# ska-sa/dc_sand

Measured on AMD Instinct MI355X. Metric: Gcoeff/s (complex weights) 64ant x 1024beam x 32768chan per GPU, higher is better.
Workload: dtype f32

## Files before the change

dc_sand_amd/csrc/bf_beamform_i8_kernel.inc:

```
#ifndef BF_I8_WEIGHTED
#define BF_I8_WEIGHTED 0
#endif
#ifndef BF_I8_QUANT
#define BF_I8_QUANT 0
#endif
#ifndef BF_I8_POWER
#define BF_I8_POWER 0
#endif
template <int FORM, bool FULL, int NW = 4>
__global__ void __launch_bounds__(NW * 64) __attribute__((amdgpu_waves_per_eu(i8_waves_per_eu(FORM, FULL, BF_I8_QUANT))))
#if BF_I8_WEIGHTED && BF_I8_POWER
bf_beamform_i8_wp_kernel(const bf_bacc_args a, const bf_weights_args w)
#elif BF_I8_POWER
bf_beamform_i8_p_kernel(const bf_bacc_args a)
#elif BF_I8_WEIGHTED && BF_I8_QUANT
bf_beamform_i8_wq_kernel(const bf_bacc_args a, const bf_weights_args w, const bf_quant_args qa)
#elif BF_I8_QUANT
bf_beamform_i8_q_kernel(const bf_bacc_args a, const bf_quant_args qa)
#elif BF_I8_WEIGHTED
bf_beamform_i8_w_kernel(const bf_bacc_args a, const bf_weights_args w)
#else
bf_beamform_i8_kernel(const bf_bacc_args a)
#endif
{
    constexpr bool WEIGHTED = BF_I8_WEIGHTED, QUANT = BF_I8_QUANT;
#if !BF_I8_WEIGHTED
    const bf_weights_args w{};
#endif
#if !BF_I8_QUANT
    const bf_quant_args qa{};
#endif
    static_assert(NW == 4 || ((NW == 8 || NW == 16) && FORM == kStaged), "8- and 16-wave workgroups exist for the staged form only");
    static_assert(!WEIGHTED || FORM == kStaged || FORM == kChain, "weights exist for the product's forms only");
    static_assert(!QUANT || (NW == 4 && (FORM == kStaged || FORM == kChain)), "the quantiser exists for the product's forms only");
    static_assert(!BF_I8_POWER || (!BF_I8_QUANT && NW == 4 && (FORM == kStaged || FORM == kChain)), "the detector exists for the product's forms only");
    constexpr bool STAGED = FORM == kStaged, SPLIT = FORM == kSplit, CHAIN = FORM == kChain;
    extern __shared__ __attribute__((aligned(16))) char staged[];
    uint32_t bid = BACC_LOGICAL_ID(a);
    const uint32_t wave = __builtin_amdgcn_readfirstlane(threadIdx.x >> 6);
    const uint32_t lane = threadIdx.x & 63u;
    const uint32_t bg = bid % a.n_bgroups;
    bid /= a.n_bgroups;
    const uint32_t tg = bid % a.n_tgroups;
    const uint32_t c = bid / a.n_tgroups;
    const uint32_t nbt_log2 = SPLIT || CHAIN ? 0u : a.nbt_log2;
    const uint32_t nbt = 1u << nbt_log2, tpr = SPLIT ? 1u : (uint32_t)NW >> nbt_log2;
    const uint32_t bt = SPLIT ? 0u : wave & (nbt - 1u), slot = SPLIT ? 0u : wave >> nbt_log2;
    const uint32_t kc = SPLIT || CHAIN ? wave : 0u;
    const uint32_t lm = lane & 15u, lg = lane >> 4;
    const uint32_t bw = (bg * nbt + bt) * 16u;
    const uint32_t tt0 = tg * a.tiles_per_wg;
    const uint32_t tt1 = min(tt0 + a.tiles_per_wg, a.nT16);
    const uint32_t n_blocks = tt1 > tt0 + slot ? (tt1 - tt0 - slot + tpr - 1u) / tpr : 0u;
    const bool idle = bw >= a.B || n_blocks == 0u;
    if (!STAGED && !CHAIN && idle) return;
    const bool has_chunk = !(SPLIT || CHAIN) || 64u * kc < a.A;
    if (STAGED) {
        typedef __attribute__((address_space(3))) void lds_void;
        typedef const __attribute__((address_space(1))) void glb_void;
        const uint32_t bytes = (tt1 - tt0) * a.A * 32u;
        const char *src = reinterpret_cast<const char *>(a.ant) + ((uint64_t)c * a.nT16 + tt0) * a.A * 32u;
        for (uint32_t k = wave; k * 1024u < bytes; k += (uint32_t)NW)
            __builtin_amdgcn_global_load_lds((glb_void *)(src + min(k * 1024u + lane * 16u, bytes - 16u)), (lds_void *)(staged + k * 1024u),
                                             16, 0, 0);
    }

    const uint32_t fw = a.flags[0];
    const uint32_t cls = (fw >> 2) == a.epoch ? (fw & 3u) : DCS_CLASS_FAST_LOW;
    const float fChan = (float)c;
    const float D = a.k.fDenominator, y = a.k.fRcpDenominator;
    const float inv = 1.0f / kFixScale;
    float fac[4] = {inv, inv, inv, inv};
    if constexpr (WEIGHTED && STAGED) {
#pragma unroll
        for (int r = 0; r < 4; r++) fac[r] = w.gs[min(bw + (lane >> 4) + 4u * (uint32_t)r, a.B - 1u)] * inv;
    } else if constexpr (WEIGHTED && CHAIN) {
        fac[0] = w.gs[min(bw + (lane & 15u), a.B - 1u)] * inv;
    }
    float kq[4] = {0.0f, 0.0f, 0.0f, 0.0f};
    uint32_t n_clip = 0u;
    if constexpr (QUANT && STAGED) {
#pragma unroll
        for (int r = 0; r < 4; r++) kq[r] = qa.gains[min(bw + (lane >> 4) + 4u * (uint32_t)r, a.B - 1u)];
    }

    const bool shared_w = STAGED && a.share_off != 0u && tpr > 1u && cls != DCS_CLASS_SLOW;
    intx4 wre[3], wim[3];
#pragma unroll
    for (int d = 0; d < 3; d++) wre[d] = wim[d] = intx4{0, 0, 0, 0};
    bool bad_re = false, bad_im = false;
    auto make_coefficients = [&]() {
        const uint32_t beam = bw + 4u * (lm & 3u) + (lm >> 2);
        const bool beam_live = beam < a.B;
        const float *tp = a.terms + 2u * (uint64_t)min(beam, a.B - 1u);
        const float *gp = WEIGHTED ? w.gn + min(beam, a.B - 1u) : nullptr;
        auto planes = [](const uint32_t (&g)[4], uint32_t (&out)[3]) {
            const uint32_t t0 = __builtin_amdgcn_perm(g[1], g[0], 0x05010400u), t1 = __builtin_amdgcn_perm(g[1], g[0], 0x07030602u);
            const uint32_t t2 = __builtin_amdgcn_perm(g[3], g[2], 0x05010400u), t3 = __builtin_amdgcn_perm(g[3], g[2], 0x07030602u);
            out[2] = __builtin_amdgcn_perm(t2, t0, 0x05040100u);
            out[1] = __builtin_amdgcn_perm(t2, t0, 0x07060302u);
            out[0] = __builtin_amdgcn_perm(t3, t1, 0x05040100u);
        };
        auto four = [&](auto gen, auto track, uint32_t q, const floatx2 (&k4)[4], const float (&g4)[4], uint32_t (&nr)[3],
                        uint32_t (&ni)[3]) {
            uint32_t gr[4], gi[4];
#pragma unroll
            for (uint32_t z = 0; z < 4; z++) {
                float re, im;
                gen(k4[z].x, k4[z].y, re, im);
                if constexpr (WEIGHTED) re = g4[z] * re, im = g4[z] * im;
                if (decltype(track)::value) {
                    bad_re |= !(fabsf(re) <= 2.0f);
                    bad_im |= !(fabsf(im) <= 2.0f);
                }
                gr[z] = fixed_word(re), gi[z] = fixed_word(im);
            }
            planes(gr, nr), planes(gi, ni);
            if (!FULL) {
                uint32_t mask = 0;
#pragma unroll
                for (uint32_t z = 0; z < 4; z++) mask |= 64u * kc + 4u * (4u * q + z) + lg < a.A ? 0xffu << (8u * z) : 0u;
#pragma unroll
                for (int d = 0; d < 3; d++) nr[d] &= mask, ni[d] &= mask;
            }
        };
// ... 2 lines not shown
            float gw[16];
#pragma unroll
            for (uint32_t z = 0; z < 16; z++) {
                const uint32_t ant = 64u * kc + 4u * z + lg;
                if constexpr (WEIGHTED) {
                    if (decltype(unrolled)::value && z >= 4u) continue;
                    gw[z] = gp[(uint64_t)min(ant, a.A - 1u) * a.B];
                }
                kp[z] = *reinterpret_cast<const floatx2 *>(tp + 2u * (uint64_t)min(ant, a.A - 1u) * a.B);
            }
            if (decltype(unrolled)::value) {
#pragma unroll
                for (uint32_t q = 0; q < 4; q++) {
                    if constexpr (WEIGHTED) {
                        if (q < 3u) {
#pragma unroll
                            for (uint32_t z = 4u * q + 4u; z < 4u * q + 8u; z++) {
                                const uint32_t ant = 64u * kc + 4u * z + lg;
                                gw[z] = gp[(uint64_t)min(ant, a.A - 1u) * a.B];
                                kp[z] = *reinterpret_cast<const floatx2 *>(tp + 2u * (uint64_t)min(ant, a.A - 1u) * a.B);
                            }
                        }
                    }
                    if (shared_w && (q & (tpr - 1u)) != slot) continue;
                    const floatx2 k4[4] = {kp[4 * q], kp[4 * q + 1], kp[4 * q + 2], kp[4 * q + 3]};
                    float g4[4] = {};
                    if constexpr (WEIGHTED) g4[0] = gw[4 * q], g4[1] = gw[4 * q + 1], g4[2] = gw[4 * q + 2], g4[3] = gw[4 * q + 3];
                    uint32_t nr[3], ni[3];
                    four(gen, std::false_type{}, q, k4, g4, nr, ni);
                    if constexpr (CHAIN) {
                        uint32_t *cw = reinterpret_cast<uint32_t *>(staged) + (kc * 6u * 64u + lane) * 4u + q;
#pragma unroll
                        for (int d = 0; d < 3; d++) cw[(uint32_t)d * 256u] = beam_live ? nr[d] : 0u, cw[(3u + (uint32_t)d) * 256u] = beam_live ? ni[d] : 0u;
                    } else {
#pragma unroll
                        for (int d = 0; d < 3; d++) wre[d][q] = (int)nr[d], wim[d][q] = (int)ni[d];
                    }
                }
            } else {
#pragma unroll 1
                for (uint32_t q = 0; q < 4; q++) {
                    const floatx2 k4[4] = {kp[0], kp[1], kp[2], kp[3]};
                    float g4[4] = {};
                    if constexpr (WEIGHTED) {
#pragma unroll
                        for (uint32_t z = 0; z < 4; z++) g4[z] = gp[(uint64_t)min(64u * kc + 4u * (4u * q + z) + lg, a.A - 1u) * a.B];
                    }
                    uint32_t nr[3], ni[3];
                    four(gen, std::true_type{}, q, k4, g4, nr, ni);
                    if constexpr (CHAIN) {
                        uint32_t *cw = reinterpret_cast<uint32_t *>(staged) + (kc * 6u * 64u + lane) * 4u + q;
#pragma unroll
                        for (int d = 0; d < 3; d++) cw[(uint32_t)d * 256u] = beam_live ? nr[d] : 0u, cw[(3u + (uint32_t)d) * 256u] = beam_live ? ni[d] : 0u;
                    } else {
#pragma unroll
                        for (int d = 0; d < 3; d++) {
                            wre[d] = intx4{wre[d][1], wre[d][2], wre[d][3], (int)nr[d]};
                            wim[d] = intx4{wim[d][1], wim[d][2], wim[d][3], (int)ni[d]};
                        }
                    }
#pragma unroll
                    for (uint32_t z = 0; z < 12; z++) kp[z] = kp[z + 4];
                }
            }
            if (!CHAIN && !beam_live) {
#pragma unroll
                for (int d = 0; d < 3; d++) wre[d] = wim[d] = intx4{0, 0, 0, 0};
            }
        };
        if (cls == DCS_CLASS_SLOW) {
            generate([&](float kx, float ky, float &re, float &im) { coeff_slow(kx, ky, fChan, D, re, im); }, std::false_type{});
        } else {
            dispatch_fast(a.k.uDiv3Exact != 0u, cls == DCS_CLASS_FAST_LOW, [&](auto div3, auto lowdeg) {
                generate([&](float kx, float ky, float &re, float &im) {
                    coeff_fast<decltype(div3)::value, decltype(lowdeg)::value>(kx, ky, fChan, D, y, re, im);
                }, std::true_type{});
            });
        }
    };

    const char *ant8 = reinterpret_cast<const char *>(a.ant);
    const uint32_t blk_bytes = a.A * 32u;
    const uint32_t m = lm & 7u;
    const bool second = lm >= 8u;
    const uint32_t last = n_blocks - 1u;
    const uint32_t voff = lg * 32u + m * 4u;
    uint32_t cur[2][16];
    auto arrived = [&](uint32_t (&v)[16]) {
        asm volatile("" : "+v"(v[0]), "+v"(v[1]), "+v"(v[2]), "+v"(v[3]), "+v"(v[4]), "+v"(v[5]), "+v"(v[6]), "+v"(v[7]));
        asm volatile("" : "+v"(v[8]), "+v"(v[9]), "+v"(v[10]), "+v"(v[11]), "+v"(v[12]), "+v"(v[13]), "+v"(v[14]), "+v"(v[15]));
    };
    auto fetch = [&](uint32_t (&dst)[16], uint32_t blk, uint32_t kc) {
        const uint32_t blkA = min(blk, last), blkB = min(blk + 1u, last);
        if (STAGED) {
            const uint32_t at = ((second ? blkB : blkA) * tpr + slot) * blk_bytes + m * 4u;
#pragma unroll
            for (uint32_t p = 0; p < 16; p++)
                dst[p] = *reinterpret_cast<const uint32_t *>(staged + at + (FULL ? lg + 4u * p : min(lg + 4u * p, a.A - 1u)) * 32u);
// ... 179 lines not shown
        } else {
            for (uint32_t blk = 0; blk < n_blocks; blk += 4) {
                if (has_chunk) {
                    arrived(cur[0]);
                    arrived(cur[1]);
#pragma unroll
                    for (int h = 0; h < 2; h++) {
                        intx4 x[4];
                        floatx4 f[4];
                        transpose(cur[h], x);
                        contract(x, f);
                        if (SPLIT)
                            park(h, f);
                        else
                            finish(whole, blk + 2u * h, f);
                    }
                }
                if (SPLIT) {
                    __syncthreads();
                    gather(whole, 0, blk);
                    gather(whole, 1, blk + 2u);
                    __syncthreads();
                }
                __builtin_amdgcn_sched_barrier(0);
                if (has_chunk) {
                    fetch(cur[0], blk + 4u, kc);
                    fetch(cur[1], blk + 6u, kc);
                }
            }
        }
    };
    if (!STAGED && !CHAIN && has_chunk) fetch(cur[0], 0, kc);
    if (CHAIN && !idle) fetch(cur[0], 0, 0u);
    __builtin_amdgcn_sched_barrier(0);
#ifdef DCS_PROBES
    if (a.probe == 3u || a.probe == 4u) {
#pragma unroll
        for (int d = 0; d < 3; d++) wre[d] = wim[d] = intx4{(int)lane, d, 2, 1};
    } else
#endif
    if ((shared_w || CHAIN ? bw < a.B : !idle) && has_chunk) make_coefficients();
    if (cls == DCS_CLASS_SLOW) {
        const uint64_t br = __builtin_amdgcn_ballot_w64(bad_re), bi = __builtin_amdgcn_ballot_w64(bad_im);
        nan_re = (uint32_t)((br | (br >> 16) | (br >> 32) | (br >> 48)) & 0xffffu);
        nan_im = (uint32_t)((bi | (bi >> 16) | (bi >> 32) | (bi >> 48)) & 0xffffu);
    }
    if constexpr (STAGED) {
        uint32_t *wx = reinterpret_cast<uint32_t *>(staged + a.share_off) + bt * (4u * 6u * 64u) + lane;
        if (shared_w && bw < a.B) {
#pragma unroll
            for (uint32_t q = 0; q < 4; q++)
                if ((q & (tpr - 1u)) == slot) {
#pragma unroll
                    for (int d = 0; d < 3; d++) wx[(q * 6u + d) * 64u] = (uint32_t)wre[d][q], wx[(q * 6u + 3u + d) * 64u] = (uint32_t)wim[d][q];
                }
        }
        __syncthreads();
        if (idle) return;
        if (shared_w) {
#pragma unroll
            for (uint32_t q = 0; q < 4; q++)
                if ((q & (tpr - 1u)) != slot) {
#pragma unroll
                    for (int d = 0; d < 3; d++) wre[d][q] = (int)wx[(q * 6u + d) * 64u], wim[d][q] = (int)wx[(q * 6u + 3u + d) * 64u];
                }
        }
    } else if constexpr (CHAIN) {
        intx4 *coef = reinterpret_cast<intx4 *>(staged);
        uint32_t *nanw = reinterpret_cast<uint32_t *>(staged + 4u * 6u * 64u * 16u);
        if (lane == 0u) nanw[2u * wave] = has_chunk ? nan_re : 0u, nanw[2u * wave + 1u] = has_chunk ? nan_im : 0u;
        float *facw = reinterpret_cast<float *>(nanw + 8);
        if constexpr (WEIGHTED) {
            if (wave == 0u && lane < 16u) facw[lane] = fac[0];
        }
        if constexpr (QUANT) {
// ... 103 lines not shown
                    float sc_next = WEIGHTED ? facw[lg] : inv;
#pragma unroll
                    for (int r = 0; r < 4; r++) {
                        const float sc = sc_next;
                        if constexpr (WEIGHTED) {
                            if (r < 3) sc_next = facw[4u * (uint32_t)r + 4u + lg];
                        }
                        floatx4 o;
#pragma unroll
                        for (int v = 0; v < 4; v++) o[v] = fmaf((float)acc[v][0][r], 65536.0f, (float)(acc[v][1][r] * 256 + acc[v][2][r])) * sc;
                        if (nan_re | nan_im) poison(r, o);
                        if (decltype(whole)::value || bb + 4u * (uint32_t)r < a.B) store(out_of(blk, r), o);
                        __builtin_amdgcn_sched_barrier(0);
                    }
                    chunk = 0u, blk += 2u;
                } else {
                    chunk++;
                }
                s++;
            };
            while (s < n_steps) {
                step(cur[0], cur[1]);
                if (s < n_steps) step(cur[1], cur[0]);
            }
        };
        if (bw + 16u <= a.B)
            run_chain(std::true_type{});
        else
            run_chain(std::false_type{});
        if constexpr (QUANT) {
            if (qa.clips) q8_tally(qa.clips, n_clip, bb, lm, a.B);
        }
        return;
    } else if (has_chunk) {
        fetch(cur[1], 2, kc);
    }
    if (bw + 16u <= a.B)
        run(std::true_type{});
    else
        run(std::false_type{});
    if constexpr (QUANT) {
        if (qa.clips) q8_tally(qa.clips, n_clip, bb, lm, a.B);
    }
}
#undef BF_I8_WEIGHTED
#undef BF_I8_QUANT
#undef BF_I8_POWER
```

dc_sand_amd/csrc/bf_beamform_mfma.hip:

```cpp

#include "bf_kernels.h"

#include <hip/hip_runtime.h>

#include <type_traits>

#include "bf_device.h"

namespace {

__device__ __forceinline__ uint32_t xcd_grouped(uint32_t w, uint32_t total, uint32_t G) { return bf_xcd_grouped(w, total, G); }
#ifdef DCS_PROBES
__device__ __forceinline__ uint32_t probe_order(uint32_t order, uint32_t w, uint32_t total, uint32_t G, uint32_t n_sharers)
{
    if (order == 1u) return w;
    if (order >= 16u && order < 24u) return (w + (order - 16u)) % total;
    if (order == 2u) {
        const uint32_t per = total >> 3, rem = total & 7u, x = w & 7u, q = w >> 3;
        return x * per + min(x, rem) + q;
    }
    return xcd_grouped(w, total, order == 3u ? n_sharers : G);
}
#define BACC_LOGICAL_ID(a) probe_order((a).order, blockIdx.x, gridDim.x, (a).xcd_group, (a).n_bgroups)
#else
// ... 105 lines not shown
            for (uint32_t j = 0; j < nj; j++) {
                uint32_t v = cur[0];
#pragma unroll
                for (uint32_t z = 1; z < NJ; z++) v = (z == j) ? cur[z] : v;
                v &= 0u - (uint32_t)(a0 + lg + 4u * j < a.A);
                acc_re = __builtin_amdgcn_mfma_f32_16x16x4f32(wr[(size_t)j * 4u * WS], (float)(int8_t)(v & 0xffu), acc_re, 0, 0, 0);
                acc_im = __builtin_amdgcn_mfma_f32_16x16x4f32(wi[(size_t)j * 4u * WS], (float)(int8_t)(v >> 8), acc_im, 0, 0, 0);
            }
        }
        if (chunk + 1 == n_chunks) {
            floatx2 *dst = reinterpret_cast<floatx2 *>(a.beams) + ((uint64_t)c * a.nT16 + tt0 + blk * TPR + slot) * a.B * 16u + lm;
            const uint32_t bb = b0 + bt * 16u + lg * 4u;
#pragma unroll
            for (int r = 0; r < 4; r++)
                if (bb + r < a.B) dst[(uint64_t)(bb + r) * 16u] = floatx2{acc_re[r], acc_im[r]};
            acc_re = floatx4{0.0f, 0.0f, 0.0f, 0.0f};
            acc_im = floatx4{0.0f, 0.0f, 0.0f, 0.0f};
        }
#pragma unroll
        for (uint32_t j = 0; j < NJ; j++) cur[j] = nxt[j];
    }
}


typedef int intx4 __attribute__((ext_vector_type(4)));
constexpr float kFixScale = 8355711.0f;

__device__ __forceinline__ uint32_t fixed_word(float w)
{
    const float f = __builtin_amdgcn_fmed3f(w * kFixScale, -kFixScale, kFixScale);
    return ((uint32_t)(int)rintf(f) + 0x808080u) ^ 0x808080u;
}

enum { kStaged = 0, kDirect = 1, kSplit = 2, kChain = 3 };
constexpr int kChainWaves = 4;

constexpr int i8_waves_per_eu(int form, bool full, bool quant = false)
{
    return form == kSplit ? (full ? 3 : 2) : (form == kChain ? kChainWaves - (quant ? 1 : 0) : (full || form == kStaged ? 4 : 3));
}

__device__ __forceinline__ uint32_t q8_pack(const floatx4 o, float k, bool count, bool live, int r, uint32_t &n_clip)
{
    uint32_t word = 0u, n = 0u;
    bool any = false;
#pragma unroll
    for (int v = 0; v < 4; v++) {
        const float y = o[v] * k;
        const float ry = rintf(y);
        const bool clip = !(fabsf(ry) <= 127.0f);
        const float q = y != y ? -128.0f : __builtin_amdgcn_fmed3f(ry, -127.0f, 127.0f);
        word |= ((uint32_t)(int)q & 0xffu) << (8 * v);
        any |= clip;
        n += clip ? 1u : 0u;
    }
    if (count && __builtin_amdgcn_ballot_w64(any && live) != 0ull) n_clip += live ? n << (8 * r) : 0u;
    return word;
}

__device__ __forceinline__ void q8_quad_transpose(uint32_t (&d)[4], uint32_t lane)
{
    const bool b0 = (lane & 1u) != 0u, b1 = (lane & 2u) != 0u;
#pragma unroll
    for (int p = 0; p < 4; p += 2) {
        const uint32_t recv = (uint32_t)__builtin_amdgcn_update_dpp(0, (int)(b0 ? d[p] : d[p + 1]), 0xB1, 0xf, 0xf, false);
        d[p] = b0 ? recv : d[p];
        d[p + 1] = b0 ? d[p + 1] : recv;
    }
#pragma unroll
    for (int p = 0; p < 2; p++) {
        const uint32_t recv = (uint32_t)__builtin_amdgcn_update_dpp(0, (int)(b1 ? d[p] : d[p + 2]), 0x4E, 0xf, 0xf, false);
// ... 81 lines not shown
            hipLaunchKernelGGL((bf_beamform_i8_wq_kernel<FORM, FULL>), grid, block, lds, stream, a, *w, *q);
        else if (q)
            hipLaunchKernelGGL((bf_beamform_i8_q_kernel<FORM, FULL>), grid, block, lds, stream, a, *q);
        else if (w)
            hipLaunchKernelGGL((bf_beamform_i8_w_kernel<FORM, FULL>), grid, block, lds, stream, a, *w);
        if (power || q || w) return;
    }
    hipLaunchKernelGGL((bf_beamform_i8_kernel<FORM, FULL, NW>), grid, block, lds, stream, a);
}

template <int FORM, int NW = 4>
void launch_i8_form(bool full, dim3 grid, dim3 block, size_t lds, hipStream_t stream, const bf_bacc_args &a,
                    const bf_weights_args *w, const bf_quant_args *q, bool power)
{
    if (full)
        launch_i8<FORM, true, NW>(grid, block, lds, stream, a, w, q, power);
    else
        launch_i8<FORM, false, NW>(grid, block, lds, stream, a, w, q, power);
}
}

hipError_t bf_launch_beamform_acc(const bf_bacc_args &a_in, const bf_weights_args *w, const bf_quant_args *q, bool power,
                                  hipStream_t stream)
{
    bf_bacc_args a = a_in;
    if (a.A == 0 || a.B == 0 || a.C == 0 || a.nT16 == 0) return hipSuccess;
    if (a.A > 256u) return hipErrorInvalidValue;
    const bool chain = a.fp32_chain != 0u;
    if ((w || q || power) && chain) return hipErrorInvalidValue;
    if (q && power) return hipErrorInvalidValue;
    const bool wide = !chain && a.A > 64u;
    const bool split = wide && BACC_KNOB(a, unstaged) != 0u;
    const bool staged_form = !chain && a.A <= 64u && !BACC_KNOB(a, unstaged);
    int nbt = wide ? 1 : (a.B > 32u ? 4 : (a.B > 16u ? 2 : 1));
#ifdef DCS_PROBES
    if (staged_form && (a.nbt_force == 1u || a.nbt_force == 2u || a.nbt_force == 4u || a.nbt_force == 8u)) nbt = (int)a.nbt_force;
#endif
    uint32_t nw = nbt == 8 ? 8u : 4u;
#ifdef DCS_PROBES
    if (staged_form && (a.nw_force == 8u || a.nw_force == 16u) && a.nw_force >= (uint32_t)nbt) nw = a.nw_force;
#endif
    while (chain && nbt > 1 && bacc_lds_bytes(nbt, a.A) > 26u * 1024u) nbt >>= 1;
    const size_t lds = chain ? bacc_lds_bytes(nbt, a.A) : 0u;
    a.nbt_log2 = nbt == 8 ? 3u : (nbt == 4 ? 2u : (nbt == 2 ? 1u : 0u));
    a.n_bgroups = (a.B + 16u * (uint32_t)nbt - 1u) / (16u * (uint32_t)nbt);
    const uint32_t tpr = split ? 1u : nw / (uint32_t)nbt;
    const uint32_t blocks_cap = staged_form && nbt == 4 && a.n_bgroups == 1u ? 8u : 16u;
    const uint32_t max_rounds = BACC_KNOB(a, max_rounds) ? BACC_KNOB(a, max_rounds) : (chain ? 16u : (staged_form || wide ? blocks_cap / tpr : 32u));
    uint32_t tiles = (a.nT16 + tpr - 1u) / tpr * tpr;
    if (tiles > max_rounds * tpr) {
        const uint32_t parts = (a.nT16 + max_rounds * tpr - 1u) / (max_rounds * tpr);
        tiles = ((a.nT16 + parts - 1u) / parts + tpr - 1u) / tpr * tpr;
    }
    const uint64_t enough = chain ? 4096u : 5120u / nw;
    while (tiles > tpr && (uint64_t)a.C * a.n_bgroups * ((a.nT16 + tiles - 1u) / tiles) < enough) tiles = ((tiles / tpr + 1u) / 2u) * tpr;
    a.tiles_per_wg = tiles;
    a.n_tgroups = (a.nT16 + tiles - 1u) / tiles;
    a.xcd_group = wide ? a.n_bgroups : (!chain && a.n_bgroups >= 16u ? a.n_bgroups : 1u);
    const uint64_t blocks = (uint64_t)a.C * a.n_bgroups * a.n_tgroups;
    if (blocks > 0x7fffffffull) return hipErrorInvalidValue;
    const dim3 grid((uint32_t)blocks), block(64u * nw);
    if (chain) {
        if (nbt == 4)
            hipLaunchKernelGGL(bf_beamform_acc_kernel<4>, grid, block, lds, stream, a);
        else if (nbt == 2)
            hipLaunchKernelGGL(bf_beamform_acc_kernel<2>, grid, block, lds, stream, a);
        else
            hipLaunchKernelGGL(bf_beamform_acc_kernel<1>, grid, block, lds, stream, a);
        return hipGetLastError();
    }
    const bool plain = !w && !q && !power;
    if (!plain && (nw != 4u || (!staged_form && (!wide || split)))) return hipErrorInvalidValue;
    if (q && a.tiles_per_wg / tpr > 126u) return hipErrorInvalidValue;
    const bool full = a.A % 64u == 0u;
    if (staged_form) {
        size_t stage_bytes = ((size_t)a.tiles_per_wg * a.A * 32u + 1023u) / 1024u * 1024u;
        if (tpr > 1u && !BACC_KNOB(a, no_share)) {
            a.share_off = (uint32_t)stage_bytes;
            stage_bytes += (size_t)nbt * 4u * 6u * 64u * sizeof(uint32_t);
        }
#ifdef DCS_PROBES
        if (plain && a.wg_per_cu >= 1u && a.wg_per_cu <= 5u && stage_bytes < 160u * 1024u / a.wg_per_cu)
            stage_bytes = (160u * 1024u / a.wg_per_cu) & ~1023u;
        if (nw == 8u)
            launch_i8_form<kStaged, 8>(full, grid, block, stage_bytes, stream, a, w, q, power);
        else if (nw == 16u)
            launch_i8_form<kStaged, 16>(full, grid, block, stage_bytes, stream, a, w, q, power);
        else
#endif
        launch_i8_form<kStaged>(full, grid, block, stage_bytes, stream, a, w, q, power);
#ifdef DCS_PROBES
    } else if (a.A <= 64u) {
        launch_i8_form<kDirect>(full, grid, block, 0, stream, a, w, q, power);
    } else if (split) {
        launch_i8_form<kSplit>(full, grid, block, 2u * 4u * 4u * 64u * 16u, stream, a, w, q, power);
#endif
    } else {
        const size_t coef_bytes = 4u * 6u * 64u * 16u + 8u * sizeof(uint32_t) + (q ? 32u : (w ? 16u : 0u)) * sizeof(float);
        launch_i8_form<kChain>(full, grid, block, coef_bytes, stream, a, w, q, power);
    }
    return hipGetLastError();
}

hipError_t bf_launch_power_integrate(const bf_pint_args &a, hipStream_t stream)
{
    if (a.total == 0u) return hipSuccess;
    const uint64_t blocks = (a.total + 255u) / 256u;
    if (blocks > 0x7fffffffull) return hipErrorInvalidValue;
    hipLaunchKernelGGL(bf_power_integrate_kernel, dim3((uint32_t)blocks), dim3(256u), 0, stream, a);
    return hipGetLastError();
}
```

dc_sand_amd/csrc/bf_capi.hip:

```cpp

#include "../../include/dcs_beamformer.h"
#ifdef DCS_PROBES
#include "../../include/dcs_probes.h"
#endif

#include <hip/hip_runtime.h>

#include <cmath>
#include <cstdio>
#include <cstdlib>
#include <cstring>
#include <new>

#include "../../include/dcs_stream_staging.h"
#include "bf_kernels.h"
#include "bf_ctx_ext.h"
#include "bf_stream_ext.h"

static_assert(sizeof(dcs_delay_vals) == 16, "delay_vals must be 4 x fp32 (BeamformerParameters.h:61-66)");

#define DCS_TRY(expr)                          \
    do {                                       \
        hipError_t _e = (expr);                \
        if (_e != hipSuccess) return (int)_e;  \
// ... 1142 lines not shown
        if (st_alloc == DCS_OK && out.d_weights) st_alloc = ensure_weights(c, s);
        if (st_alloc != DCS_OK) return st_alloc;
    }
    float dt_coeff = 0.0f;
    int st = fill_dt(c, src, 0, 1, &dt_coeff);
    if (st != DCS_OK) return st;
    uint32_t epoch = 0;
    st = launch_bform_terms(c, out.d_weights, 1, nullptr, dt_coeff, nullptr, s, &epoch);
    if (st != DCS_OK) return st;
    bf_bacc_args a;
    std::memset(&a, 0, sizeof(a));
    a.terms = c->d_terms;
    a.flags = c->d_flags;
    a.epoch = epoch;
    a.ant = d_antenna;
    a.beams = static_cast<float *>(d_beams);
    a.A = A;
    a.B = B;
    a.C = C;
    a.nT16 = nt / 16u;
    a.k = c->k;
    a.fp32_chain = (c->tune.math_mode & 8) ? 1u : 0u;
#ifdef DCS_PROBES
    auto knob = [](int32_t v, const char *env) { const char *e = std::getenv(env); return (uint32_t)(v ? v : (e ? std::atoi(e) : 0)); };
    a.max_rounds = knob(c->probe.bacc_rounds, "DCS_BACC_ROUNDS");
    a.probe = knob(c->probe.bacc_probe, "DCS_BACC_PROBE");
    a.unstaged = knob(c->probe.bacc_unstaged, "DCS_BACC_UNSTAGED");
    a.plain_stores = knob(c->probe.bacc_plain, "DCS_BACC_PLAIN");
    a.no_share = knob(c->probe.bacc_no_share, "DCS_BACC_NOSHARE");
    a.wg_per_cu = knob(c->probe.bacc_wg_per_cu, "DCS_BACC_WPC");
    a.order = knob(c->probe.bacc_order, "DCS_BACC_ORDER");
    a.nbt_force = knob(c->probe.bacc_nbt, "DCS_BACC_NBT");
    a.nw_force = knob(c->probe.bacc_waves, "DCS_BACC_WAVES");
#endif
    const bf_weights_args wa = {out.d_weights, c->d_wnorm, c->d_wscale};
    return (int)bf_launch_beamform_acc(a, out.d_weights ? &wa : nullptr, out.kind == bacc_output::kInt8 ? &out.quant : nullptr,
                                       out.kind == bacc_output::kBlockPower, s);
}

int generate_and_beamform_weighted_impl(dcs_bf_context *c, const float *dt, uint64_t t0, uint32_t nt, const int8_t *d_antenna,
                                        size_t antenna_bytes, const float *d_weights, float *d_beams, size_t beams_bytes,
                                        void *stream)
{
    if (!c || !weights_ok(d_weights)) return DCS_ERR_INVALID_ARGUMENT;
    if (!dt && t0 % 16u) return DCS_ERR_INVALID_ARGUMENT;
    return beamform_impl(c, dt_or_index(dt, t0), nt, d_antenna, antenna_bytes, d_beams, beams_bytes, stream, d_weights);
}

int beamform_accumulated_weighted_impl(dcs_bf_context *c, const float *dt_coeff, uint64_t t_coeff, uint32_t nt,
                                       const int8_t *d_antenna, size_t antenna_bytes, const float *d_weights, float *d_beams,
                                       size_t beams_bytes, void *stream)
{
    if (!c || !weights_ok(d_weights)) return DCS_ERR_INVALID_ARGUMENT;
    return beamform_acc_impl(c, dt_or_index(dt_coeff, t_coeff), nt, d_antenna, antenna_bytes, d_beams, beams_bytes,
                             stream, {bacc_output::kFloat, d_weights, {}});
}

int beamform_accumulated_q8_impl(dcs_bf_context *c, const float *dt_coeff, uint64_t t_coeff, uint32_t nt, const int8_t *d_antenna,
                                 size_t antenna_bytes, const float *d_weights, const float *d_quant_gains, int8_t *d_beams_q8,
                                 size_t beams_bytes, unsigned long long *d_clip_count, void *stream)
{
    if (!c || !weights_ok(d_quant_gains) || (d_weights && !weights_ok(d_weights)) || (reinterpret_cast<uintptr_t>(d_clip_count) & 7u))
        return DCS_ERR_INVALID_ARGUMENT;
    return beamform_acc_impl(c, dt_or_index(dt_coeff, t_coeff), nt, d_antenna, antenna_bytes, d_beams_q8, beams_bytes,
                             stream, {bacc_output::kInt8, d_weights, {d_quant_gains, d_clip_count}});
}
// ... 678 lines not shown
```

dc_sand_amd/csrc/bf_kernels.h:

```cpp
#ifndef DCS_BF_KERNELS_H
#define DCS_BF_KERNELS_H

#include <hip/hip_runtime.h>
#include <stdint.h>

#include "bf_math.h"

struct bf_tiled_args {
    const dcs_delay_vals *delays;
    void *out;
    const float *dt_dev;
    float dt0;
    uint32_t n_pairs;
    uint32_t c0, nc;
    uint32_t nt;
    uint32_t chan_per_block;
    uint32_t n_tile_groups;
    uint32_t n_cblocks;
    uint32_t xcd_remap;
#ifdef DCS_PROBES
    uint32_t pace;
#endif
    dcs_bf_consts k;
    const float *terms;
// ... 79 lines not shown
    const float *terms;
    const uint32_t *flags;
    uint32_t epoch;
    const int8_t *ant;
    float *beams;
    uint32_t A, B, C;
    uint32_t nt16;
    uint32_t tex0;
    uint32_t nt16_total;
    uint32_t chan_per_block;
    uint32_t n_bgroups, n_cblocks;
    dcs_bf_consts k;
};
hipError_t bf_launch_beamform(const bf_beamform_args &a, const bf_weights_args *w, hipStream_t stream);

struct bf_bacc_args {
    const float *terms;
    const uint32_t *flags;
    uint32_t epoch;
    const int8_t *ant;
    float *beams;
    uint32_t A, B, C, nT16;
    uint32_t fp32_chain;
    uint32_t share_off;
#ifdef DCS_PROBES
    uint32_t max_rounds;
    uint32_t no_share;
    uint32_t plain_stores;
    uint32_t wg_per_cu;
    uint32_t unstaged;
    uint32_t order;
    uint32_t nbt_force;
    uint32_t nw_force;
    uint32_t probe;
#endif
    uint32_t tiles_per_wg, n_bgroups, n_tgroups, nbt_log2, xcd_group;
    dcs_bf_consts k;
};
__host__ __device__ inline uint32_t bf_xcd_grouped(uint32_t w, uint32_t total, uint32_t G)
{
    if (G <= 1u) return w;
    const uint32_t full = total - total % (8u * G);
    if (w >= full) return w;
    const uint32_t x = w & 7u, q = w >> 3;
    return ((q / G) * 8u + x) * G + q % G;
}

#ifdef DCS_PROBES
#define BACC_KNOB(a, f) ((a).f)
#else
#define BACC_KNOB(a, f) 0u
#endif
struct bf_quant_args {
    const float *gains;
    unsigned long long *clips;
};
hipError_t bf_launch_beamform_acc(const bf_bacc_args &a, const bf_weights_args *w, const bf_quant_args *q, bool power,
                                  hipStream_t stream);
struct bf_pint_args {
    const float *block_power;
    float *spectra;
    uint64_t total;
    uint32_t B, C;
    uint32_t nr_blocks;
    uint32_t n;
    uint32_t accumulate;
// ... 83 lines not shown
```

include/dcs_probes.h:

```cpp
#ifndef DCS_PROBES_H
#define DCS_PROBES_H

#include "dcs_beamformer.h"

#ifdef __cplusplus
extern "C" {
#endif
#pragma GCC visibility push(default)

struct dcs_probe_knobs {
    int32_t nomath;
    int32_t pace;
    int32_t fail_at_step;
    int32_t bacc_probe;
    int32_t bacc_rounds;
    int32_t bacc_no_share;
    int32_t bacc_plain;
    int32_t bacc_wg_per_cu;
    int32_t bacc_unstaged;
    int32_t bacc_order;
    int32_t bacc_nbt;
    int32_t bacc_waves;
};
int dcs_probe_set_knobs(dcs_bf_context *ctx, const struct dcs_probe_knobs *k);

int dcs_probe_sincos(int which, const float *d_x, size_t n, float *d_sin, float *d_cos, void *stream);
int dcs_probe_fill(void *d_out, size_t bytes, int nontemporal, void *stream);
int dcs_probe_store_pattern(void *d_out, uint32_t rows, uint32_t cols_kib, uint32_t qb, uint32_t rb, int order,
                            int xcd_remap, int nontemporal, uint32_t block_threads, void *stream);

int dcs_probe_one_store(void *d_out, size_t bytes, int store_mode, int stores_per_thread, uint32_t row_bytes, void *stream);

int dcs_probe_reduce(const void *d_in, size_t bytes, uint64_t *checksum, float *max_modulus_dev, void *stream);

int dcs_probe_mfma(int which, uint32_t blocks, uint32_t iters, float *d_out, void *stream);

uint32_t dcs_probe_xcd_grouped(uint32_t w, uint32_t total, uint32_t group);

int dcs_probe_copy(const void *d_in, void *d_out, size_t bytes, int store_mode, int per_thread, void *stream);

#pragma GCC visibility pop
#ifdef __cplusplus
}
#endif
#endif
```

probes/dcs_probes.py:

```python
from __future__ import annotations

import ctypes
from ctypes import POINTER, byref, c_float, c_int, c_size_t, c_uint32, c_uint64, c_void_p

import numpy as np

from .build import LIB, build

_VP = c_void_p
SIGNATURES = [
    ("dcs_probe_sincos", c_int, [c_int, _VP, c_size_t, _VP, _VP, _VP]),
    ("dcs_probe_fill", c_int, [_VP, c_size_t, c_int, _VP]),
    ("dcs_probe_copy", c_int, [_VP, _VP, c_size_t, c_int, c_int, _VP]),
    ("dcs_probe_one_store", c_int, [_VP, c_size_t, c_int, c_int, c_uint32, _VP]),
    ("dcs_probe_reduce", c_int, [_VP, c_size_t, POINTER(c_uint64), POINTER(c_float), _VP]),
    ("dcs_probe_mfma", c_int, [c_int, c_uint32, c_uint32, _VP, _VP]),
    ("dcs_probe_store_pattern", c_int, [_VP, c_uint32, c_uint32, c_uint32, c_uint32, c_int, c_int, c_int, c_uint32, _VP]),
    ("dcs_probe_set_knobs", c_int, [_VP, _VP]),
    ("dcs_probe_xcd_grouped", c_uint32, [c_uint32, c_uint32, c_uint32]),
]

KNOB_FIELDS = ("nomath", "pace", "fail_at_step", "bacc_probe", "bacc_rounds", "bacc_no_share", "bacc_plain", "bacc_wg_per_cu",
               "bacc_unstaged", "bacc_order", "bacc_nbt", "bacc_waves")

_LIB = None


def lib() -> ctypes.CDLL:
    global _LIB
    if _LIB is None:
        if not LIB.exists():
            build()
        L = ctypes.CDLL(str(LIB))
        for name, restype, argtypes in SIGNATURES:
            fn = getattr(L, name)
            fn.restype = restype
            fn.argtypes = argtypes
        _LIB = L
    return _LIB


def _check(status: int, where: str) -> None:
    if status != 0:
        raise RuntimeError(f"{where}: status {status}")


def _s(stream) -> c_void_p:
    if stream is None:
        return c_void_p(None)
    return c_void_p(int(getattr(stream, "handle", stream)))


def tensor_properties(d_ptr, nbytes: int, stream=None) -> tuple[int, float]:
    ck = c_uint64(0)
    dev = c_float(0.0)
    _check(lib().dcs_probe_reduce(c_void_p(int(d_ptr)), int(nbytes), byref(ck), byref(dev), _s(stream)), "dcs_probe_reduce")
# ... 45 lines not shown
```

Measured before the change: 934.2.

## Add two-beam-tile chain form reusing each antenna fetch across 32 beams

Adds a kChain2 kernel form for the wide-antenna plain float path. Each workgroup builds coefficient images for two 16-beam tiles in LDS and runs MFMAs for both tiles on every transposed antenna chunk, so each antenna load is shared across twice as many beams. The launcher selects it by default when B>16 and no weights, quantiser or detector are used, and adjusts tiles-per-wg and the grid-size threshold to match. In exchange it doubles accumulator registers and LDS and lowers the occupancy target to 3 waves per EU.

```diff
diff --git a/dc_sand_amd/csrc/bf_beamform_i8_kernel.inc b/dc_sand_amd/csrc/bf_beamform_i8_kernel.inc
--- a/dc_sand_amd/csrc/bf_beamform_i8_kernel.inc
+++ b/dc_sand_amd/csrc/bf_beamform_i8_kernel.inc
@@ -34,7 +34,8 @@
     static_assert(!WEIGHTED || FORM == kStaged || FORM == kChain, "weights exist for the product's forms only");
     static_assert(!QUANT || (NW == 4 && (FORM == kStaged || FORM == kChain)), "the quantiser exists for the product's forms only");
     static_assert(!BF_I8_POWER || (!BF_I8_QUANT && NW == 4 && (FORM == kStaged || FORM == kChain)), "the detector exists for the product's forms only");
-    constexpr bool STAGED = FORM == kStaged, SPLIT = FORM == kSplit, CHAIN = FORM == kChain;
+    static_assert(FORM != kChain2 || (NW == 4 && !BF_I8_WEIGHTED && !BF_I8_QUANT && !BF_I8_POWER), "the two-tile form exists for the plain float call only");
+    constexpr bool STAGED = FORM == kStaged, SPLIT = FORM == kSplit, CHAIN = FORM == kChain, CHAIN2 = FORM == kChain2;
     extern __shared__ __attribute__((aligned(16))) char staged[];
     uint32_t bid = BACC_LOGICAL_ID(a);
     const uint32_t wave = __builtin_amdgcn_readfirstlane(threadIdx.x >> 6);
@@ -43,18 +44,18 @@
     bid /= a.n_bgroups;
     const uint32_t tg = bid % a.n_tgroups;
     const uint32_t c = bid / a.n_tgroups;
-    const uint32_t nbt_log2 = SPLIT || CHAIN ? 0u : a.nbt_log2;
+    const uint32_t nbt_log2 = SPLIT || CHAIN || CHAIN2 ? 0u : a.nbt_log2;
     const uint32_t nbt = 1u << nbt_log2, tpr = SPLIT ? 1u : (uint32_t)NW >> nbt_log2;
     const uint32_t bt = SPLIT ? 0u : wave & (nbt - 1u), slot = SPLIT ? 0u : wave >> nbt_log2;
-    const uint32_t kc = SPLIT || CHAIN ? wave : 0u;
+    const uint32_t kc = SPLIT || CHAIN || CHAIN2 ? wave : 0u;
     const uint32_t lm = lane & 15u, lg = lane >> 4;
-    const uint32_t bw = (bg * nbt + bt) * 16u;
+    const uint32_t bw = CHAIN2 ? bg * 32u : (bg * nbt + bt) * 16u;
     const uint32_t tt0 = tg * a.tiles_per_wg;
     const uint32_t tt1 = min(tt0 + a.tiles_per_wg, a.nT16);
     const uint32_t n_blocks = tt1 > tt0 + slot ? (tt1 - tt0 - slot + tpr - 1u) / tpr : 0u;
     const bool idle = bw >= a.B || n_blocks == 0u;
-    if (!STAGED && !CHAIN && idle) return;
-    const bool has_chunk = !(SPLIT || CHAIN) || 64u * kc < a.A;
+    if (!STAGED && !CHAIN && !CHAIN2 && idle) return;
+    const bool has_chunk = !(SPLIT || CHAIN || CHAIN2) || 64u * kc < a.A;
     if (STAGED) {
         typedef __attribute__((address_space(3))) void lds_void;
         typedef const __attribute__((address_space(1))) void glb_void;
@@ -89,8 +90,10 @@
 #pragma unroll
     for (int d = 0; d < 3; d++) wre[d] = wim[d] = intx4{0, 0, 0, 0};
     bool bad_re = false, bad_im = false;
-    auto make_coefficients = [&]() {
-        const uint32_t beam = bw + 4u * (lm & 3u) + (lm >> 2);
+    auto make_coefficients = [&](auto tile) {
+        uint32_t tile_bw;
+        if constexpr (CHAIN2) tile_bw = tile.bw; else tile_bw = bw;
+        const uint32_t beam = tile_bw + 4u * (lm & 3u) + (lm >> 2);
         const bool beam_live = beam < a.B;
         const float *tp = a.terms + 2u * (uint64_t)min(beam, a.B - 1u);
         const float *gp = WEIGHTED ? w.gn + min(beam, a.B - 1u) : nullptr;
@@ -159,6 +162,10 @@
                         uint32_t *cw = reinterpret_cast<uint32_t *>(staged) + (kc * 6u * 64u + lane) * 4u + q;
 #pragma unroll
                         for (int d = 0; d < 3; d++) cw[(uint32_t)d * 256u] = beam_live ? nr[d] : 0u, cw[(3u + (uint32_t)d) * 256u] = beam_live ? ni[d] : 0u;
+                    } else if constexpr (CHAIN2) {
+                        uint32_t *cw = reinterpret_cast<uint32_t *>(tile.image) + (kc * 6u * 64u + lane) * 4u + q;
+#pragma unroll
+                        for (int d = 0; d < 3; d++) cw[(uint32_t)d * 256u] = beam_live ? nr[d] : 0u, cw[(3u + (uint32_t)d) * 256u] = beam_live ? ni[d] : 0u;
                     } else {
 #pragma unroll
                         for (int d = 0; d < 3; d++) wre[d][q] = (int)nr[d], wim[d][q] = (int)ni[d];
@@ -179,6 +186,10 @@
                         uint32_t *cw = reinterpret_cast<uint32_t *>(staged) + (kc * 6u * 64u + lane) * 4u + q;
 #pragma unroll
                         for (int d = 0; d < 3; d++) cw[(uint32_t)d * 256u] = beam_live ? nr[d] : 0u, cw[(3u + (uint32_t)d) * 256u] = beam_live ? ni[d] : 0u;
+                    } else if constexpr (CHAIN2) {
+                        uint32_t *cw = reinterpret_cast<uint32_t *>(tile.image) + (kc * 6u * 64u + lane) * 4u + q;
+#pragma unroll
+                        for (int d = 0; d < 3; d++) cw[(uint32_t)d * 256u] = beam_live ? nr[d] : 0u, cw[(3u + (uint32_t)d) * 256u] = beam_live ? ni[d] : 0u;
                     } else {
 #pragma unroll
                         for (int d = 0; d < 3; d++) {
@@ -190,7 +201,7 @@
                     for (uint32_t z = 0; z < 12; z++) kp[z] = kp[z + 4];
                 }
             }
-            if (!CHAIN && !beam_live) {
+            if (!CHAIN && !CHAIN2 && !beam_live) {
 #pragma unroll
                 for (int d = 0; d < 3; d++) wre[d] = wim[d] = intx4{0, 0, 0, 0};
             }
@@ -436,6 +447,8 @@
     };
     if (!STAGED && !CHAIN && has_chunk) fetch(cur[0], 0, kc);
     if (CHAIN && !idle) fetch(cur[0], 0, 0u);
+    if (CHAIN2 && !idle) fetch(cur[0], 0, 0u);
+    const bool live1 = CHAIN2 && bw + 16u < a.B;
     __builtin_amdgcn_sched_barrier(0);
 #ifdef DCS_PROBES
     if (a.probe == 3u || a.probe == 4u) {
@@ -443,8 +456,25 @@
         for (int d = 0; d < 3; d++) wre[d] = wim[d] = intx4{(int)lane, d, 2, 1};
     } else
 #endif
-    if ((shared_w || CHAIN ? bw < a.B : !idle) && has_chunk) make_coefficients();
-    if (cls == DCS_CLASS_SLOW) {
+    if constexpr (CHAIN2) {
+        uint32_t *nanw = reinterpret_cast<uint32_t *>(staged + 2u * kChainImage);
+#pragma unroll 1
+        for (uint32_t t = 0; t < 2u; t++) {
+            uint32_t nr = 0u, ni = 0u;
+            if (has_chunk && (t == 0u || live1)) {
+                bad_re = bad_im = false;
+                make_coefficients(i8_tile_at{bw + 16u * t, staged + t * kChainImage});
+                if (cls == DCS_CLASS_SLOW) {
+                    const uint64_t br = __builtin_amdgcn_ballot_w64(bad_re), bi = __builtin_amdgcn_ballot_w64(bad_im);
+                    nr = (uint32_t)((br | (br >> 16) | (br >> 32) | (br >> 48)) & 0xffffu);
+                    ni = (uint32_t)((bi | (bi >> 16) | (bi >> 32) | (bi >> 48)) & 0xffffu);
+                }
+            }
+            if (lane == 0u) nanw[2u * (4u * t + wave)] = nr, nanw[2u * (4u * t + wave) + 1u] = ni;
+        }
+    } else
+    if ((shared_w || CHAIN ? bw < a.B : !idle) && has_chunk) make_coefficients(i8_one_tile{});
+    if (!CHAIN2 && cls == DCS_CLASS_SLOW) {
         const uint64_t br = __builtin_amdgcn_ballot_w64(bad_re), bi = __builtin_amdgcn_ballot_w64(bad_im);
         nan_re = (uint32_t)((br | (br >> 16) | (br >> 32) | (br >> 48)) & 0xffffu);
         nan_im = (uint32_t)((bi | (bi >> 16) | (bi >> 32) | (bi >> 48)) & 0xffffu);
@@ -614,6 +644,74 @@
             if (qa.clips) q8_tally(qa.clips, n_clip, bb, lm, a.B);
         }
         return;
+    } else if constexpr (CHAIN2) {
+        const intx4 *coef = reinterpret_cast<const intx4 *>(staged);
+        const uint32_t *nanw = reinterpret_cast<const uint32_t *>(staged + 2u * kChainImage);
+        __syncthreads();
+        if (idle) return;
+        uint32_t nan2[2][2];
+#pragma unroll
+        for (uint32_t t = 0; t < 2u; t++) {
+            nan2[t][0] = nanw[8u * t] | nanw[8u * t + 2u] | nanw[8u * t + 4u] | nanw[8u * t + 6u];
+            nan2[t][1] = nanw[8u * t + 1u] | nanw[8u * t + 3u] | nanw[8u * t + 5u] | nanw[8u * t + 7u];
+        }
+        const uint32_t n_chunks = (a.A + 63u) / 64u;
+        auto out_of_tile = [&](uint32_t blk, int r, uint32_t tbb) {
+            const uint32_t blkB = min(blk + 1u, last);
+            char *base = out8 + ((uint64_t)c * a.nT16 + tt0 + blk * tpr + slot) * out_blk;
+            return reinterpret_cast<floatx4 *>(base + ((second ? (blkB - blk) * tpr * out_blk : 0u) + tbb * 128u + m * 16u + 512u * r));
+        };
+        auto run_chain2 = [&](auto whole) {
+            intx4 acc[2][4][3];
+            uint32_t f_chunk = 1u % n_chunks, f_blk = 2u * (1u / n_chunks);
+            auto step = [&](auto first, uint32_t chunk) {
+                arrived(cur[0]);
+                intx4 x[4];
+                transpose(cur[0], x);
+                __builtin_amdgcn_sched_barrier(0);
+                fetch(cur[0], f_blk, f_chunk);
+                if (++f_chunk == n_chunks) f_chunk = 0u, f_blk += 2u;
+#pragma unroll
+                for (int t = 0; t < 2; t++) {
+                    if (t == 1 && !live1) break;
+#pragma unroll
+                    for (int half = 0; half < 2; half++) {
+#pragma unroll
+                        for (int d = 0; d < 3; d++) {
+                            const intx4 w = coef[((4u * (uint32_t)t + chunk) * 6u + 3u * (uint32_t)half + (uint32_t)d) * 64u + lane];
+#pragma unroll
+                            for (int v = half; v < 4; v += 2)
+                                acc[t][v][d] = __builtin_amdgcn_mfma_i32_16x16x64_i8(w, x[v], decltype(first)::value ? zero : acc[t][v][d], 0, 0, 0);
+                        }
+                    }
+                }
+            };
+            for (uint32_t blk = 0; blk < n_blocks; blk += 2u) {
+                step(std::true_type{}, 0u);
+#pragma unroll 1
+                for (uint32_t chunk = 1u; chunk < n_chunks; chunk++) step(std::false_type{}, chunk);
+#pragma unroll
+                for (int t = 0; t < 2; t++) {
+                    if (t == 1 && !live1) break;
+                    nan_re = nan2[t][0], nan_im = nan2[t][1];
+                    const uint32_t tbb = bb + 16u * (uint32_t)t;
+#pragma unroll
+                    for (int r = 0; r < 4; r++) {
+                        floatx4 o;
+#pragma unroll
+                        for (int v = 0; v < 4; v++) o[v] = fmaf((float)acc[t][v][0][r], 65536.0f, (float)(acc[t][v][1][r] * 256 + acc[t][v][2][r])) * inv;
+                        if (nan_re | nan_im) poison(r, o);
+                        if (decltype(whole)::value || tbb + 4u * (uint32_t)r < a.B) store(out_of_tile(blk, r, tbb), o);
+                        __builtin_amdgcn_sched_barrier(0);
+                    }
+                }
+            }
+        };
+        if (bw + 32u <= a.B)
+            run_chain2(std::true_type{});
+        else
+            run_chain2(std::false_type{});
+        return;
     } else if (has_chunk) {
         fetch(cur[1], 2, kc);
     }
diff --git a/dc_sand_amd/csrc/bf_beamform_mfma.hip b/dc_sand_amd/csrc/bf_beamform_mfma.hip
--- a/dc_sand_amd/csrc/bf_beamform_mfma.hip
+++ b/dc_sand_amd/csrc/bf_beamform_mfma.hip
@@ -161,11 +161,19 @@
     return ((uint32_t)(int)rintf(f) + 0x808080u) ^ 0x808080u;
 }
 
-enum { kStaged = 0, kDirect = 1, kSplit = 2, kChain = 3 };
+enum { kStaged = 0, kDirect = 1, kSplit = 2, kChain = 3, kChain2 = 4 };
 constexpr int kChainWaves = 4;
+constexpr int kChain2Waves = 3;
+constexpr uint32_t kChainImage = 4u * 6u * 64u * 16u;
+struct i8_one_tile {};
+struct i8_tile_at {
+    uint32_t bw;
+    char *image;
+};
 
 constexpr int i8_waves_per_eu(int form, bool full, bool quant = false)
 {
+    if (form == kChain2) return kChain2Waves;
     return form == kSplit ? (full ? 3 : 2) : (form == kChain ? kChainWaves - (quant ? 1 : 0) : (full || form == kStaged ? 4 : 3));
 }
 
@@ -313,7 +321,8 @@
     const bool wide = !chain && a.A > 64u;
     const bool split = wide && BACC_KNOB(a, unstaged) != 0u;
     const bool staged_form = !chain && a.A <= 64u && !BACC_KNOB(a, unstaged);
-    int nbt = wide ? 1 : (a.B > 32u ? 4 : (a.B > 16u ? 2 : 1));
+    const bool two = wide && !split && !w && !q && !power && a.B > 16u && !BACC_KNOB(a, one_tile) && !BACC_KNOB(a, probe);
+    int nbt = two ? 2 : (wide ? 1 : (a.B > 32u ? 4 : (a.B > 16u ? 2 : 1)));
 #ifdef DCS_PROBES
     if (staged_form && (a.nbt_force == 1u || a.nbt_force == 2u || a.nbt_force == 4u || a.nbt_force == 8u)) nbt = (int)a.nbt_force;
 #endif
@@ -325,7 +334,7 @@
     const size_t lds = chain ? bacc_lds_bytes(nbt, a.A) : 0u;
     a.nbt_log2 = nbt == 8 ? 3u : (nbt == 4 ? 2u : (nbt == 2 ? 1u : 0u));
     a.n_bgroups = (a.B + 16u * (uint32_t)nbt - 1u) / (16u * (uint32_t)nbt);
-    const uint32_t tpr = split ? 1u : nw / (uint32_t)nbt;
+    const uint32_t tpr = split ? 1u : (two ? nw : nw / (uint32_t)nbt);
     const uint32_t blocks_cap = staged_form && nbt == 4 && a.n_bgroups == 1u ? 8u : 16u;
     const uint32_t max_rounds = BACC_KNOB(a, max_rounds) ? BACC_KNOB(a, max_rounds) : (chain ? 16u : (staged_form || wide ? blocks_cap / tpr : 32u));
     uint32_t tiles = (a.nT16 + tpr - 1u) / tpr * tpr;
@@ -333,7 +342,7 @@
         const uint32_t parts = (a.nT16 + max_rounds * tpr - 1u) / (max_rounds * tpr);
         tiles = ((a.nT16 + parts - 1u) / parts + tpr - 1u) / tpr * tpr;
     }
-    const uint64_t enough = chain ? 4096u : 5120u / nw;
+    const uint64_t enough = chain ? 4096u : (two ? 768u : 5120u / nw);
     while (tiles > tpr && (uint64_t)a.C * a.n_bgroups * ((a.nT16 + tiles - 1u) / tiles) < enough) tiles = ((tiles / tpr + 1u) / 2u) * tpr;
     a.tiles_per_wg = tiles;
     a.n_tgroups = (a.nT16 + tiles - 1u) / tiles;
@@ -376,6 +385,8 @@
     } else if (split) {
         launch_i8_form<kSplit>(full, grid, block, 2u * 4u * 4u * 64u * 16u, stream, a, w, q, power);
 #endif
+    } else if (two) {
+        launch_i8_form<kChain2>(full, grid, block, 2u * kChainImage + 16u * sizeof(uint32_t), stream, a, w, q, power);
     } else {
         const size_t coef_bytes = 4u * 6u * 64u * 16u + 8u * sizeof(uint32_t) + (q ? 32u : (w ? 16u : 0u)) * sizeof(float);
         launch_i8_form<kChain>(full, grid, block, coef_bytes, stream, a, w, q, power);
diff --git a/dc_sand_amd/csrc/bf_capi.hip b/dc_sand_amd/csrc/bf_capi.hip
--- a/dc_sand_amd/csrc/bf_capi.hip
+++ b/dc_sand_amd/csrc/bf_capi.hip
@@ -1198,6 +1198,7 @@
     a.order = knob(c->probe.bacc_order, "DCS_BACC_ORDER");
     a.nbt_force = knob(c->probe.bacc_nbt, "DCS_BACC_NBT");
     a.nw_force = knob(c->probe.bacc_waves, "DCS_BACC_WAVES");
+    a.one_tile = knob(c->probe.bacc_one_tile, "DCS_BACC_ONE_TILE");
 #endif
     const bf_weights_args wa = {out.d_weights, c->d_wnorm, c->d_wscale};
     return (int)bf_launch_beamform_acc(a, out.d_weights ? &wa : nullptr, out.kind == bacc_output::kInt8 ? &out.quant : nullptr,
diff --git a/dc_sand_amd/csrc/bf_kernels.h b/dc_sand_amd/csrc/bf_kernels.h
--- a/dc_sand_amd/csrc/bf_kernels.h
+++ b/dc_sand_amd/csrc/bf_kernels.h
@@ -135,6 +135,7 @@
     uint32_t order;
     uint32_t nbt_force;
     uint32_t nw_force;
+    uint32_t one_tile;
     uint32_t probe;
 #endif
     uint32_t tiles_per_wg, n_bgroups, n_tgroups, nbt_log2, xcd_group;
diff --git a/include/dcs_probes.h b/include/dcs_probes.h
--- a/include/dcs_probes.h
+++ b/include/dcs_probes.h
@@ -21,6 +21,7 @@
     int32_t bacc_order;
     int32_t bacc_nbt;
     int32_t bacc_waves;
+    int32_t bacc_one_tile;
 };
 int dcs_probe_set_knobs(dcs_bf_context *ctx, const struct dcs_probe_knobs *k);
 
diff --git a/probes/dcs_probes.py b/probes/dcs_probes.py
--- a/probes/dcs_probes.py
+++ b/probes/dcs_probes.py
@@ -21,7 +21,7 @@
 ]
 
 KNOB_FIELDS = ("nomath", "pace", "fail_at_step", "bacc_probe", "bacc_rounds", "bacc_no_share", "bacc_plain", "bacc_wg_per_cu",
-               "bacc_unstaged", "bacc_order", "bacc_nbt", "bacc_waves")
+               "bacc_unstaged", "bacc_order", "bacc_nbt", "bacc_waves", "bacc_one_tile")
 
 _LIB = None
 
```

New measurement: 927.9. About the same (-0.7%).
